# opencb/hpg-variant

Measured on AMD Instinct MI355X. Metric: variants/s chi2 assoc, higher is better.
Workload: dtype u8

## Files before the change

### hpg-variant_amd/csrc/hpgv_capi.hip

```cpp
#include "hpgv_internal.h"
#include <cstdlib>

extern "C" {

const char *hpgv_version(void) { return "hpgv-mi355x 0.1 (gfx950)"; }

int hpgv_device_count(void) {
    int n = 0;
    if (hipGetDeviceCount(&n) != hipSuccess) return -1;
    return n;
}

const char *hpgv_last_error(const hpgv_ctx *ctx) { return ctx ? ctx->err.c_str() : g_create_error.c_str(); }

static void read_environment(hpgv_ctx *ctx) {
    auto num = [](const char *name, long lo, long hi, long *out) { const char *e = getenv(name); if (e && *e) { long v = atol(e); *out = v < lo ? lo : v > hi ? hi : v; } };
    num("HPGV_BATCH_COPY", 0, 1, &ctx->batch_copy);
    num("HPGV_BATCH_FUSED", 0, 1, &ctx->batch_fused);
    num("HPGV_STATS_ALL2", 0, 1, &ctx->stats_all2);
    num("HPGV_ASSOC_ROWS", 0, 1, &ctx->assoc_rows);
    num("HPGV_PINNED_NONCOHERENT", 0, 1, &ctx->pinned_noncoherent);
    num("HPGV_VMM_TRACE", 0, 1, &ctx->vmm_trace);
    num("HPGV_DECODE_TILES", 0, 1, &ctx->decode_tiles);
#ifdef HPGV_ABLATION
// ... 120 lines not shown
    }
    ctx->tok_scratch.clear();
    for (auto &r : ctx->grow) grow_release(r);
    ctx->grow.clear();
    hpgv_epi_release(ctx->epi);
    for (Slot *s : ctx->slots) {
        s->release();
        if (s->stream) (void)hipStreamDestroy(s->stream);
        delete s;
    }
    for (int i = 0; i < 4; ++i) if (ctx->ev[i]) (void)hipEventDestroy(ctx->ev[i]);
    delete ctx;
}

#ifdef HPGV_ABLATION
#define HPGV_SHIPPED_ONLY(ok, what)
#else
#define HPGV_SHIPPED_ONLY(ok, what) if (!(ok)) return fail(ctx, HPGV_ERR_UNSUPPORTED, what ": that form is an ablation build's (-DHPGV_ABLATION, tools/build_ablation.py)");
#endif

int hpgv_set_option(hpgv_ctx *ctx, const char *key, long value) {
    if (is_group(ctx) && key && !strcmp(key, "group_self_exchange")) { ctx->group_self_exchange = value ? 1 : 0; return HPGV_OK; }
    GROUP_ALL(ctx, hpgv_set_option(m_, key, value))
    if (!ctx || !key) return HPGV_ERR_INVALID;
    if (!strcmp(key, "row_align")) {
        if (value < 16 || (value & (value - 1))) return fail(ctx, HPGV_ERR_INVALID, "row_align must be a power of two >= 16");
        if (ctx->assoc.set || ctx->tdt.set || ctx->stats.set)
            return fail(ctx, HPGV_ERR_STATE, "row_align must be set before the cohort");
        ctx->row_align = value;
    } else if (!strcmp(key, "row_pad")) {
        if (value < 0 || value % 16 || value > 65536) return fail(ctx, HPGV_ERR_INVALID, "row_pad must be a multiple of 16 in [0, 65536]");
        if (ctx->assoc.set || ctx->tdt.set || ctx->stats.set)
            return fail(ctx, HPGV_ERR_STATE, "row_pad must be set before the cohort");
        ctx->row_pad = value;
    } else if (!strcmp(key, "variants_per_wave")) {
        if (value < 1 || value > 1024) return fail(ctx, HPGV_ERR_INVALID, "variants_per_wave out of range");
        ctx->vpw = value;
    } else if (!strcmp(key, "nontemporal")) {
        HPGV_SHIPPED_ONLY(value != 0, "nontemporal = 0")
        ctx->nontemporal = value ? 1 : 0;
    } else if (!strcmp(key, "profile")) {
        ctx->profile = value ? 1 : 0;
    } else if (!strcmp(key, "scan_unroll")) {
        if (value != 4 && value != 8 && value != 10 && value != 12 && value != 16)
            return fail(ctx, HPGV_ERR_INVALID, "scan_unroll must be one of 4, 8, 10, 12, 16");
        HPGV_SHIPPED_ONLY(value == 4, "scan_unroll other than 4")
        ctx->scan_unroll = value;
    } else if (!strcmp(key, "pipeline")) {
        HPGV_SHIPPED_ONLY(value != 0, "pipeline = 0")
        ctx->pipeline = value ? 1 : 0;
    } else if (!strcmp(key, "fisher_cut_exp")) {
        if (value < 12 || value > 300) return fail(ctx, HPGV_ERR_INVALID, "fisher_cut_exp must be in [12, 300]");
        ctx->fisher_cut_exp = value;
    } else if (!strcmp(key, "epi_complete")) {
        ctx->epi_complete = value ? 1 : 0;
    } else if (!strcmp(key, "epi_triples_mfma")) {
        ctx->epi_triples_mfma = value ? 1 : 0;
    } else if (!strcmp(key, "epi_pairs_mfma")) {
        ctx->epi_pairs_mfma = value ? 1 : 0;
    } else if (!strcmp(key, "epi_wide")) {
        if (value < 0 || value > 2) return fail(ctx, HPGV_ERR_INVALID, "epi_wide must be 0 (the packed kernels' limits), 1 (the wide kernel where the shape needs it) or 2 (the wide kernel for every listed-combination launch)");
        ctx->epi_wide = value;
    } else if (!strcmp(key, "epi_triples_1pass")) {
        if (value < 0 || value > 2) return fail(ctx, HPGV_ERR_INVALID, "epi_triples_1pass must be 0 (two passes), 1 (the cells nine at a time) or 2 (one pass, one wave per SIMD)");
        HPGV_SHIPPED_ONLY(value != 2, "epi_triples_1pass = 2")
        ctx->epi_triples_1pass = value;
    } else if (!strcmp(key, "scan_lds")) {
        if (value < 0 || value > 160 * 1024) return fail(ctx, HPGV_ERR_INVALID, "scan_lds must be in [0, 163840]");
        ctx->scan_lds = value;
    } else if (!strcmp(key, "batch_copy")) {
        ctx->batch_copy = value ? 1 : 0;
    } else if (!strcmp(key, "inflate_wave")) {
        if (value < 0 || value > 4) return fail(ctx, HPGV_ERR_INVALID, "inflate_wave must be 0 (lane per block), 1 (by the number of blocks), 2 (wave per block), 4 (wave per block, several symbols per round) or 3 (lane per block, symbol tables in LDS)");
        HPGV_SHIPPED_ONLY(value == 1 || value == 4, "inflate_wave other than 1 / 4 (a wave per block, several symbols per round)")
        ctx->inflate_wave = value;
    } else if (!strcmp(key, "tokenizer_tiles")) {
        if (value < 0 || value > 2) return fail(ctx, HPGV_ERR_INVALID, "tokenizer_tiles must be 2 (one sweep), 1 (two sweeps) or 0 (line by line)");
        HPGV_SHIPPED_ONLY(value == 1, "tokenizer_tiles other than 1 (two sweeps)")
        ctx->tokenizer_tiles = value;
    } else if (!strcmp(key, "fisher_width")) {
        if (value != 64 && value != 32 && value != 16 && value != 8) return fail(ctx, HPGV_ERR_INVALID, "fisher_width must be 64, 32, 16 or 8");
        HPGV_SHIPPED_ONLY(value == 16, "fisher_width other than 16")
        ctx->fisher_width = value;
    } else if (!strcmp(key, "batch_fused")) {
        ctx->batch_fused = value ? 1 : 0;
    } else if (!strcmp(key, "pipe_waves")) {
        if (value != 4 && value != 6 && value != 8) return fail(ctx, HPGV_ERR_INVALID, "pipe_waves must be 4, 6 or 8");
        HPGV_SHIPPED_ONLY(value == 4, "pipe_waves other than 4")
        ctx->pipe_waves = value;
    } else if (!strcmp(key, "persistent")) {
        HPGV_SHIPPED_ONLY(value == 0, "persistent = 1")
        ctx->persistent = value ? 1 : 0;
    } else if (!strcmp(key, "part_aligned_loads")) {
        HPGV_SHIPPED_ONLY(value == 0, "part_aligned_loads = 1")
        ctx->part_aligned = value ? 1 : 0;
    } else if (!strcmp(key, "blocks_per_cu")) {
        if (value < 1 || value > 8) return fail(ctx, HPGV_ERR_INVALID, "blocks_per_cu must be in 1..8");
        ctx->blocks_per_cu = value;
    } else {
        return fail(ctx, HPGV_ERR_INVALID, "unknown option '%s'", key);
    }
    return HPGV_OK;
}


int hpgv_set_cohort(hpgv_ctx *ctx, const uint8_t *condition, int n_samples) {
    HPGV_ABI_TRY
    GROUP_ALL(ctx, hpgv_set_cohort(m_, condition, n_samples))
    if (!ctx) return HPGV_ERR_INVALID;
    if (!condition || n_samples < 0) return fail(ctx, HPGV_ERR_INVALID, "bad cohort arguments");
    DeviceGuard g(ctx->device);
    int nA = 0, nU = 0;
    for (int j = 0; j < n_samples; ++j) {
        if (condition[j] == HPGV_COND_AFFECTED) nA++;
        else if (condition[j] == HPGV_COND_UNAFFECTED) nU++;
    }
    size_t segA = round_up((size_t)nA, 16), segU = round_up((size_t)nU, 16);
    size_t pitch = round_up(segA + segU, (size_t)ctx->row_align) + (size_t)ctx->row_pad;
    if (pitch == 0) pitch = (size_t)ctx->row_align;
    if (!pitch_supported(pitch)) return fail(ctx, HPGV_ERR_UNSUPPORTED, "cohort of %d samples exceeds the row-length limit", n_samples);
    Layout &L = ctx->assoc;
    L.n_samples = n_samples;
    L.pitch = pitch;
    L.col_of_pos.assign(pitch, -1);
    size_t a = 0, u = segA;
    for (int j = 0; j < n_samples; ++j) {
        if (condition[j] == HPGV_COND_AFFECTED) L.col_of_pos[a++] = j;
        else if (condition[j] == HPGV_COND_UNAFFECTED) L.col_of_pos[u++] = j;
    }
    ctx->nA = nA; ctx->nU = nU; ctx->chunksA = (int)(segA / 16);
    {
        std::vector<uint8_t> cond(round_up((size_t)n_samples, 16) + 16, (uint8_t)HPGV_COND_OTHER);
        for (int j = 0; j < n_samples; ++j) cond[(size_t)j] = condition[j] == HPGV_COND_AFFECTED ? 1 : condition[j] == HPGV_COND_UNAFFECTED ? 0 : 2;
        HIPCHK(ctx, ctx->d_cond.reserve(cond.size()));
        HIPCHK(ctx, hipMemcpy(ctx->d_cond.p, cond.data(), cond.size(), hipMemcpyHostToDevice));
    }
    return upload_layout(ctx, L);
    HPGV_ABI_CATCH(ctx)
}

int hpgv_assoc_layout(const hpgv_ctx *ctx, int *n_affected, int *n_unaffected, size_t *pitch) {
    ctx = first_member(ctx);
    if (!ctx) return HPGV_ERR_INVALID;
    if (!ctx->assoc.set) return fail(ctx, HPGV_ERR_STATE, "hpgv_set_cohort has not been called");
    if (n_affected) *n_affected = ctx->nA;
    if (n_unaffected) *n_unaffected = ctx->nU;
    if (pitch) *pitch = ctx->assoc.pitch;
    return HPGV_OK;
}

int hpgv_set_logfact(hpgv_ctx *ctx, const double *table, size_t n) {
    GROUP_ALL(ctx, hpgv_set_logfact(m_, table, n))
    if (!ctx) return HPGV_ERR_INVALID;
    if (!table || n == 0) return fail(ctx, HPGV_ERR_INVALID, "empty log-factorial table");
    DeviceGuard g(ctx->device);
    ctx->n_lf = 0;
    if (ctx->cap_lf < n) {
        if (ctx->d_lf_base) { (void)hipFree(ctx->d_lf_base); ctx->d_lf_base = nullptr; ctx->d_lf = nullptr; ctx->cap_lf = 0; }
        HIPCHK(ctx, hipMalloc(&ctx->d_lf_base, (n + 4) * sizeof(double)));
        HIPCHK(ctx, hipMemset(ctx->d_lf_base, 0, (n + 4) * sizeof(double)));
        ctx->d_lf = ctx->d_lf_base + 2;
        ctx->cap_lf = n;
    }
    HIPCHK(ctx, hipMemcpy(ctx->d_lf, table, n * sizeof(double), hipMemcpyHostToDevice));
    ctx->n_lf = n;
    return HPGV_OK;
// ... 415 lines not shown
```

### hpg-variant_amd/csrc/hpgv_internal.h

```cpp
#pragma once
#include "../../include/hpgv.h"
#include "hpgv_kernels.h"
#include "hpgv_tdt_stats_kernels.h"
#include "hpgv_epi_kernels.h"

#include <hip/hip_runtime.h>
#include <cctype>

#include <algorithm>
#include <atomic>
#include <cmath>
#include <cstdarg>
#include <cstdio>
#include <cstring>
#include <mutex>
#include <new>
#include <string>
#include <vector>

namespace { thread_local std::string g_create_error; }

struct DevBuf {
    void *p = nullptr;
    size_t cap = 0;
// ... 71 lines not shown
    }
};

struct TextMeta {
    char *base;
    size_t max_lines;
    TextMeta(const DevBuf &meta, int max_lines_) : base(meta.as<char>()), max_lines((size_t)max_lines_) {}
    static size_t bytes(int max_lines) { return 16 + ((size_t)max_lines + 2) * sizeof(uint64_t) + (size_t)max_lines * 10 * sizeof(uint32_t) + 16; }
    int *n_lines() const { return (int *)base; }
    unsigned long long *line_off() const { return (unsigned long long *)(base + 16); }
    uint32_t *field_off() const { return (uint32_t *)(base + 16 + (max_lines + 2) * sizeof(uint64_t)); }
};

struct Staged {
    const uint8_t *d_raw = nullptr;
    size_t raw_pitch = 0;
    const uint8_t *d_laid = nullptr;
    int which = 0;
    const uint8_t *d_isx = nullptr;
    int n = 0;
    size_t out_stride = 0;
    bool text = false;
};

struct EpiState {
    bool have_data = false, have_folds = false;
    int V = 0, nA = 0, nU = 0, num_folds = 0, W = 0, V_alloc = 0, n_chunks = 0;
    bool wide_only = false;
    int fold_cap = 0;
    int rank_fold_cap = 0;
    uint8_t *d_data = nullptr;
    uint32_t *d_planes = nullptr;
    uint32_t rev_off = 0;
    hpgv_epi_rank_info rank_info{};
    uint32_t *d_marg = nullptr;
    bool complete = false;
    hpgv::EpiChunk *d_chunks = nullptr;
    uint32_t *d_chunk_cls = nullptr;
    hpgv::EpiFold *d_folds = nullptr;
    uint32_t *d_group_w0 = nullptr;
    std::vector<int32_t> group_size;
    DevBuf cand;
    unsigned *d_cand_count = nullptr;
    unsigned cand_cap = 0;
    double *d_thr = nullptr;
    DevBuf tile_base;
};

struct hpgv_ctx {
    std::vector<hpgv_ctx *> members;
    hpgv_ctx *parent = nullptr;
    struct GroupState *grp = nullptr;
    long group_self_exchange = 0;
    std::atomic<unsigned> deal_next{0};
    std::atomic<int> in_flight{0};
    int device = 0;
    mutable std::string err;
    std::mutex mu;
    long row_align = 16;
    long row_pad = 0;
    long vpw = 2;
    long nontemporal = 1;
    long profile = 0;
    std::mutex alias_mu;
    std::vector<std::pair<const char *, const char *>> text_alias;
    struct TextTiles { const char *d_text, *d_base; const void *d_tiles; uint64_t n_tiles; };
    std::vector<TextTiles> text_tiles;
    struct TextHeld { const char *host_text; Slot *slot; const char *d_text; const unsigned long long *d_line_off; int n_lines; };
    std::vector<TextHeld> text_held;
    long part_aligned = 0;
    long scan_unroll = 4;
    long persistent = 0;
    long blocks_per_cu = 8;
    long pipeline = 1;
    long pipe_waves = 4;
    long fisher_cut_exp = 22;
    long epi_complete = 1;
    long epi_pairs_mfma = 1;
    long epi_triples_mfma = 1;
    long epi_wide = 0;
    long epi_triples_1pass = 1;
    long scan_lds = 0;
    long fisher_width = 16;
    long inflate_wave = 1;
    long tokenizer_tiles = 1;
    long batch_copy = 0;
    long batch_fused = 1;
    long batch_lds_max = 65536;
    long stats_all2 = 1;
    long assoc_rows = 1;
    long pinned_noncoherent = 0;
    long vmm_trace = 0;
    long decode_tiles = 1;
#ifdef HPGV_ABLATION
    long stats_rows = 0, stats_bs = 0, stats_debug = 0;
    long fisher_lds = 0;
    long inflate_lds_pad = 0, inflate_wave_wgs = 0, inflate_lane_wgs = 0;
#endif
    int n_cus = 256;
    Layout assoc;
    int nA = 0, nU = 0, chunksA = 0;
    DevBuf d_cond;
    Layout tdt;
    hpgv::TdtPlan tdt_plan;
    Layout stats;
    Layout sgroups;
    std::vector<uint32_t> sg_off;
    std::vector<int> sg_size;
    DevBuf d_sg_chunks;
    DevBuf d_group_of_col;
    bool all_grouped = false;
    Layout mendel;
    int mendel_trios = 0, mendel_pchunks = 0;
    hpgv::MendelLuts mendel_luts{};
    uint8_t *d_mendel_male = nullptr;
    double *d_lf = nullptr;
    double *d_lf_base = nullptr;
    size_t n_lf = 0;
    size_t cap_lf = 0;
    DevBuf d_thr;
    hipEvent_t ev[4] = {nullptr, nullptr, nullptr, nullptr};
    bool have_scan_ev = false, have_stats_ev = false;
    std::vector<Slot *> slots;
    uint32_t *d_sink = nullptr;
    uint32_t *d_crc_tab = nullptr;
    struct TokScratch {
        hipStream_t stream = nullptr;
        DevBuf blocks, line_off, extra;
    };
    std::mutex tok_mu;
    std::vector<TokScratch *> tok_scratch;
    struct GrowRange { char *base = nullptr; size_t reserved = 0, committed = 0; std::vector<hipMemGenericAllocationHandle_t> pieces; std::vector<size_t> sizes; };
    std::vector<GrowRange> grow;
    double filt_min_maf = -1.0, filt_max_missing = -1.0;
    long filt_max_mendel = -1;
    double filt_min_dom = -1.0, filt_min_rec = -1.0;
    std::mutex epi_mu;
    EpiState epi;
};

namespace {

[[maybe_unused]] int fail(const hpgv_ctx *ctx, int code, const char *fmt, ...) {
    char buf[512];
    va_list ap;
    va_start(ap, fmt);
    vsnprintf(buf, sizeof buf, fmt, ap);
    va_end(ap);
    if (ctx) {
        ctx->err = buf;
        if (ctx->parent) {
            std::lock_guard<std::mutex> lk(ctx->parent->mu);
            ctx->parent->err = buf;
        }
    } else g_create_error = buf;
    return code;
}

#define HPGV_ABI_TRY try {
#define HPGV_ABI_CATCH(ctx)                                                                         \
    } catch (const std::bad_alloc &) { return fail(ctx, HPGV_ERR_NOMEM, "out of host memory"); }     \
      catch (...) { return fail(ctx, HPGV_ERR_INVALID, "unexpected C++ exception inside the engine"); }

inline bool is_group(const hpgv_ctx *c) { return c && !c->members.empty(); }
inline hpgv_ctx *first_member(hpgv_ctx *c) { return is_group(c) ? c->members[0] : c; }
inline const hpgv_ctx *first_member(const hpgv_ctx *c) { return is_group(c) ? c->members[0] : c; }
// ... 136 lines not shown
```

### hpg-variant_amd/csrc/hpgv_kernels.h

```cpp
#pragma once
#include <hip/hip_runtime.h>
#include <stdint.h>

namespace hpgv {

__device__ __forceinline__ uint32_t nib_nonzero(uint32_t x) {
    uint32_t y = x | (x << 1);
    y = y | (y << 2);
    return y & 0x88888888u;
}
__device__ __forceinline__ uint32_t nib_not_f(uint32_t x) { return nib_nonzero(~x); }

__device__ __forceinline__ int wave_sum(int v) {
    v += __builtin_amdgcn_update_dpp(0, v, 0xB1, 0xF, 0xF, true);
    v += __builtin_amdgcn_update_dpp(0, v, 0x4E, 0xF, 0xF, true);
    v += __builtin_amdgcn_update_dpp(0, v, 0x141, 0xF, 0xF, true);
    v += __builtin_amdgcn_update_dpp(0, v, 0x140, 0xF, 0xF, true);
    return __builtin_amdgcn_readlane(v, 0) + __builtin_amdgcn_readlane(v, 16) +
           __builtin_amdgcn_readlane(v, 32) + __builtin_amdgcn_readlane(v, 48);
}

template <bool NT>
__device__ __forceinline__ uint4 load16(const uint4 *p);
template <bool NT>
// ... 159 lines not shown
    const uint8_t *g0 = gt + (size_t)v_begin * pitch;
    AssocAcc acc = {0u, 0u, 0u};
    uint4 qa[U], qb[U];
    assoc_issue_tile<NT, U>(qa, g0, pitch, 0, ipr, chunks, lane);
    for (int t = 0; t < n_tiles; t += 2) {
        if (t + 1 < n_tiles) assoc_issue_tile<NT, U>(qb, g0, pitch, t + 1, ipr, chunks, lane);
        acc = assoc_consume_tile<U>(qa, acc, t, ipr, v_begin, lane, chunksA, TA, TU, is_x, counts);
        if (t + 1 < n_tiles) {
            if (t + 2 < n_tiles) assoc_issue_tile<NT, U>(qa, g0, pitch, t + 2, ipr, chunks, lane);
            acc = assoc_consume_tile<U>(qb, acc, t + 1, ipr, v_begin, lane, chunksA, TA, TU, is_x, counts);
        }
    }
}

__device__ __forceinline__ double chisq_p_value(double x) {
    if (x != x) return x;
    if (x <= 0.0) return 1.0;
    const double y = x / 2.0;
    double P;
    if (y > 0.5) P = 1.0 - erfc(sqrt(y));
    else         P = erf(sqrt(y));
    return 1.0 - P;
}

__device__ __forceinline__ double assoc_odds(int A1, int A2, int U1, int U2) {
    return (A2 == 0 || U1 == 0) ? __builtin_nan("") : ((double)A1 / A2) * ((double)U2 / U1);
}

__device__ __forceinline__ double assoc_chisq_value(int a, int c, int b, int d) {
    const double total = a + c + b + d;
    const double t_aff = a + c, t_un = b + d, t_1 = a + b, t_2 = c + d;
    const double e_a1 = (t_aff * t_1) / total;
    const double e_a2 = (t_aff * t_2) / total;
    const double e_u1 = (t_un * t_1) / total;
    const double e_u2 = (t_un * t_2) / total;
    return ((a - e_a1) * (a - e_a1)) / e_a1 + ((c - e_a2) * (c - e_a2)) / e_a2 +
           ((b - e_u1) * (b - e_u1)) / e_u1 + ((d - e_u2) * (d - e_u2)) / e_u2;
}

static __global__ __launch_bounds__(256) void k_assoc_chisq(const int4 *__restrict__ counts, int n,
                                                     double *__restrict__ odds,
                                                     double *__restrict__ chisq,
                                                     double *__restrict__ pval) {
    const int i = blockIdx.x * blockDim.x + threadIdx.x;
    if (i >= n) return;
    const int4 c4 = counts[i];
    const int a = c4.x, c = c4.y, b = c4.z, d = c4.w;
    const double x = assoc_chisq_value(a, c, b, d);
    odds[i] = assoc_odds(a, c, b, d);
    chisq[i] = x;
    pval[i] = chisq_p_value(x);
}

__device__ __forceinline__ double wave_sum_f64(double v) {
#pragma unroll
    for (int off = 32; off > 0; off >>= 1) v += __shfl_xor(v, off);
    return v;
}
__device__ __forceinline__ double wave_max_f64(double v) {
#pragma unroll
    for (int off = 32; off > 0; off >>= 1) { const double o = __shfl_xor(v, off); v = o > v ? o : v; }
    return v;
}

__device__ const double k_exp2_j64[64] = {
    0x1.0000000000000p+0, 0x1.02c9a3e778061p+0, 0x1.059b0d3158574p+0, 0x1.0874518759bc8p+0,
    0x1.0b5586cf9890fp+0, 0x1.0e3ec32d3d1a2p+0, 0x1.11301d0125b51p+0, 0x1.1429aaea92de0p+0,
    0x1.172b83c7d517bp+0, 0x1.1a35beb6fcb75p+0, 0x1.1d4873168b9aap+0, 0x1.2063b88628cd6p+0,
    0x1.2387a6e756238p+0, 0x1.26b4565e27cddp+0, 0x1.29e9df51fdee1p+0, 0x1.2d285a6e4030bp+0,
    0x1.306fe0a31b715p+0, 0x1.33c08b26416ffp+0, 0x1.371a7373aa9cbp+0, 0x1.3a7db34e59ff7p+0,
    0x1.3dea64c123422p+0, 0x1.4160a21f72e2ap+0, 0x1.44e086061892dp+0, 0x1.486a2b5c13cd0p+0,
    0x1.4bfdad5362a27p+0, 0x1.4f9b2769d2ca7p+0, 0x1.5342b569d4f82p+0, 0x1.56f4736b527dap+0,
    0x1.5ab07dd485429p+0, 0x1.5e76f15ad2148p+0, 0x1.6247eb03a5585p+0, 0x1.6623882552225p+0,
    0x1.6a09e667f3bcdp+0, 0x1.6dfb23c651a2fp+0, 0x1.71f75e8ec5f74p+0, 0x1.75feb564267c9p+0,
    0x1.7a11473eb0187p+0, 0x1.7e2f336cf4e62p+0, 0x1.82589994cce13p+0, 0x1.868d99b4492edp+0,
    0x1.8ace5422aa0dbp+0, 0x1.8f1ae99157736p+0, 0x1.93737b0cdc5e5p+0, 0x1.97d829fde4e50p+0,
    0x1.9c49182a3f090p+0, 0x1.a0c667b5de565p+0, 0x1.a5503b23e255dp+0, 0x1.a9e6b5579fdbfp+0,
    0x1.ae89f995ad3adp+0, 0x1.b33a2b84f15fbp+0, 0x1.b7f76f2fb5e47p+0, 0x1.bcc1e904bc1d2p+0,
    0x1.c199bdd85529cp+0, 0x1.c67f12e57d14bp+0, 0x1.cb720dcef9069p+0, 0x1.d072d4a07897cp+0,
    0x1.d5818dcfba487p+0, 0x1.da9e603db3285p+0, 0x1.dfc97337b9b5fp+0, 0x1.e502ee78b3ff6p+0,
    0x1.ea4afa2a490dap+0, 0x1.efa1bee615a27p+0, 0x1.f50765b6e4540p+0, 0x1.fa7c1819e90d8p+0,
};
__device__ __forceinline__ double fisher_exp(double e, const double *tab ) {
    const double kf = __builtin_rint(e * 0x1.71547652b82fep+6);
    double r = __builtin_fma(-kf, 0x1.62e42fe000000p-7, e);
    r = __builtin_fma(-kf, 0x1.f473de6af278fp-36, r);
    const int ki = (int)kf;
    const double tj = tab[ki & 63];
    double q = __builtin_fma(r, 1.0 / 120.0, 1.0 / 24.0);
    q = __builtin_fma(r, q, 1.0 / 6.0);
    q = __builtin_fma(r, q, 0.5);
    q = __builtin_fma(r * r, q, r);
    const double y = __builtin_fma(tj, q, tj);
    return e < -1100.0 ? 0.0 : __builtin_ldexp(y, ki >> 6);
}

struct FisherTab {
    const double *lf; const double *xt ; double konst; int r1, c1, d0;
    __device__ __forceinline__ double at(uint32_t byte_off) const { return *reinterpret_cast<const double *>(reinterpret_cast<const char *>(lf) + byte_off); }
    __device__ __forceinline__ double e(int x) const {
        const uint32_t x8 = (uint32_t)x << 3;
        return konst - at(x8) - at(((uint32_t)r1 << 3) - x8) - at(((uint32_t)c1 << 3) - x8) - at(((uint32_t)d0 << 3) + x8);
    }
    __device__ __forceinline__ double p(int x) const { return fisher_exp(e(x), xt); }
    __device__ __forceinline__ void e2(int x, double *e0, double *e1) const {
        const char *b = reinterpret_cast<const char *>(lf) - 16;
        double2 q0, q1, q2, q3;
        __builtin_memcpy(&q0, b + ((uint32_t)(x + 2) << 3), 16);
        __builtin_memcpy(&q1, b + ((uint32_t)(r1 - x + 1) << 3), 16);
        __builtin_memcpy(&q2, b + ((uint32_t)(c1 - x + 1) << 3), 16);
        __builtin_memcpy(&q3, b + ((uint32_t)(d0 + x + 2) << 3), 16);
        *e0 = konst - q0.x - q1.y - q2.y - q3.x;
        *e1 = konst - q0.y - q1.x - q2.x - q3.y;
    }
};

template <int W> __device__ __forceinline__ int sub_lane(int lane) { return lane & (W - 1); }
template <int W> __device__ __forceinline__ uint64_t sub_ballot(bool pred, int lane) {
    const uint64_t b = __ballot(pred);
    if constexpr (W == 64) { (void)lane; return b; }
    else return (b >> (lane & ~(W - 1))) & ((1ull << W) - 1ull);
}
template <int W> __device__ __forceinline__ double sub_sum_f64(double v) {
#pragma unroll
    for (int off = W / 2; off > 0; off >>= 1) v += __shfl_xor(v, off);
    return v;
}
template <int W> __device__ __forceinline__ double sub_first_f64(double v, int lane) { return __shfl(v, lane & ~(W - 1)); }

template <int W>
__device__ __forceinline__ void fisher_boundaries(const FisherTab &T, double thr , int L1, int R1, int L2, int R2, int lane,
                                                  int *xL, int *xR) {
    const int sl = sub_lane<W>(lane);
    while (R1 - L1 > W || R2 - L2 > W) {
        const bool go1 = R1 - L1 > W, go2 = R2 - L2 > W;
        const int step1 = (R1 - L1 + W - 1) / W, step2 = (R2 - L2 + W - 1) / W;
        const int x1 = L1 + sl * step1, x2 = L2 + sl * step2;
        const double v1 = (go1 && x1 < R1) ? T.e(x1) : 0.0;
        const double v2 = (go2 && x2 < R2) ? T.e(x2) : 0.0;
        if (go1) {
            const int j = __builtin_popcountll(sub_ballot<W>(x1 < R1 && v1 <= thr, lane));
            const int xj = L1 + j * step1;
            const int nL = (j == 0) ? L1 : L1 + (j - 1) * step1 + 1, nR = (j == W || xj >= R1) ? R1 : xj;
            L1 = nL; R1 = nR;
        }
        if (go2) {
            const int j = __builtin_popcountll(sub_ballot<W>(x2 < R2 && v2 > thr, lane));
            const int xj = L2 + j * step2;
            const int nL = (j == 0) ? L2 : L2 + (j - 1) * step2 + 1, nR = (j == W || xj >= R2) ? R2 : xj;
            L2 = nL; R2 = nR;
        }
    }
    const int x1 = L1 + sl, x2 = L2 + sl;
    const double v1 = x1 < R1 ? T.e(x1) : 0.0, v2 = x2 < R2 ? T.e(x2) : 0.0;
    *xL = L1 + __builtin_popcountll(sub_ballot<W>(x1 < R1 && v1 <= thr, lane));
    *xR = L2 + __builtin_popcountll(sub_ballot<W>(x2 < R2 && v2 > thr, lane));
}

template <int W>
__device__ __forceinline__ double fisher_tails(const FisherTab &T, int xL, int xR, int lo, int hi, int lane, double rel_cut) {
    const int sl = sub_lane<W>(lane);
    double partL = 0.0, partR = 0.0, cutL = 0.0, cutR = 0.0;
    bool onL = true, onR = true;
    for (int k = 0; onL || onR; ++k) {
        const int firstL = xL - 1 - 2 * W * k, firstR = xR + 2 * W * k;
        if (firstL < lo) onL = false;
        if (firstR > hi) onR = false;
        const int a = firstL - 2 * sl, b = firstR + 2 * sl;
        double eL0 = -2000.0, eL1 = -2000.0, eR0 = -2000.0, eR1 = -2000.0;
        if (onL && a >= lo) { double lo_e, hi_e; T.e2(a - 1, &lo_e, &hi_e); eL0 = hi_e; if (a - 1 >= lo) eL1 = lo_e; }
        if (onR && b <= hi) { double lo_e, hi_e; T.e2(b, &lo_e, &hi_e); eR0 = lo_e; if (b + 1 <= hi) eR1 = hi_e; }
        const double sL0 = fisher_exp(eL0, T.xt), sL1 = fisher_exp(eL1, T.xt), sR0 = fisher_exp(eR0, T.xt), sR1 = fisher_exp(eR1, T.xt);
        partL += sL0 + sL1; partR += sR0 + sR1;
        if (k == 0) { cutL = rel_cut * sub_first_f64<W>(sL0, lane); cutR = rel_cut * sub_first_f64<W>(sR0, lane); }
        if (onL && sub_ballot<W>(sL0 > cutL || sL1 > cutL, lane) == 0ull) onL = false;
        if (onR && sub_ballot<W>(sR0 > cutR || sR1 > cutR, lane) == 0ull) onR = false;
    }
    return sub_sum_f64<W>(partL + partR);
}

template <int W>
__device__ __forceinline__ bool fisher_boundary_windows(const FisherTab &T, double thr , int mode, int obs, int lane,
                                                        int *L1, int *R1, int *L2, int *R2) {
    const int sl = sub_lane<W>(lane);
    const int g1 = obs <= mode ? obs + 1 : 2 * mode - obs + 1, g2 = obs <= mode ? 2 * mode - obs : obs;
    int w1 = g1 - W / 2, w2 = g2 - W / 2;
    w1 = w1 > *R1 - W ? *R1 - W : w1; w1 = w1 < *L1 ? *L1 : w1;
    w2 = w2 > *R2 - W ? *R2 - W : w2; w2 = w2 < *L2 ? *L2 : w2;
    const int x1 = w1 + sl, x2 = w2 + sl;
    const bool in1 = x1 < *R1, in2 = x2 < *R2;
    const double v1 = in1 ? T.e(x1) : 0.0, v2 = in2 ? T.e(x2) : 0.0;
    const int n1 = __builtin_popcountll(sub_ballot<W>(in1, lane)), n2 = __builtin_popcountll(sub_ballot<W>(in2, lane));
    const int c1 = __builtin_popcountll(sub_ballot<W>(in1 && v1 <= thr, lane)), c2 = __builtin_popcountll(sub_ballot<W>(in2 && v2 > thr, lane));
    bool ok = true;
    if (c1 == 0 && w1 > *L1) { *R1 = w1; ok = false; }
    else if (c1 == n1 && w1 + n1 < *R1) { *L1 = w1 + n1; ok = false; }
    else { *L1 = w1 + c1; *R1 = w1 + c1; }
    if (c2 == 0 && w2 > *L2) { *R2 = w2; ok = false; }
    else if (c2 == n2 && w2 + n2 < *R2) { *L2 = w2 + n2; ok = false; }
    else { *L2 = w2 + c2; *R2 = w2 + c2; }
    return ok;
}

template <int W>
__device__ __forceinline__ double fisher_sub(int a, int b, int c, int d, const double *__restrict__ lf,
                                             const double *exp_tab , double rel_cut, int lane) {
    const int sl = sub_lane<W>(lane);
    const int r1 = a + b, r2 = c + d, c1 = a + c, nn = r1 + r2;
    const int lo = (c1 - r2) > 0 ? (c1 - r2) : 0;
    const int hi = r1 < c1 ? r1 : c1;
    FisherTab T;
    T.lf = lf; T.xt = exp_tab; T.r1 = r1; T.c1 = c1; T.d0 = r2 - c1;
    T.konst = lf[r1] + lf[r2] + lf[c1] + lf[nn - c1] - lf[nn];
    const double thr = T.e(a) + 9.9999995000000333e-08;
    double sum;
    if (hi - lo < 8 * W) {
        double part = 0.0;
        for (int x = lo + sl; x <= hi; x += W) {
            const double ex = T.e(x);
            if (ex <= thr) part += fisher_exp(ex, exp_tab);
        }
        sum = sub_sum_f64<W>(part);
    } else {
        const double prod = (double)(r1 + 1) * (double)(c1 + 1), den = (double)(nn + 2);
        double md = __builtin_floor(prod / den);
        const double rem = __builtin_fma(-md, den, prod);
        md += rem >= den ? 1.0 : (rem < 0.0 ? -1.0 : 0.0);
        int mode = (int)md;
        mode = mode < lo ? lo : (mode > hi ? hi : mode);
        int L1 = lo, R1 = mode + 1, L2 = mode + 1, R2 = hi + 1, xL, xR;
        if (fisher_boundary_windows<W>(T, thr, mode, a, lane, &L1, &R1, &L2, &R2)) { xL = L1; xR = L2; }
        else fisher_boundaries<W>(T, thr, L1, R1, L2, R2, lane, &xL, &xR);
        sum = fisher_tails<W>(T, xL, xR, lo, hi, lane, rel_cut);
    }
    return sum > 1.0 ? 1.0 : sum;
}

__device__ __forceinline__ double fisher_wave(int a, int b, int c, int d, const double *__restrict__ lf,
                                              const double *exp_tab , double rel_cut, int lane) {
    return fisher_sub<64>(a, b, c, d, lf, exp_tab, rel_cut, lane);
}

template <int W>
__global__ __launch_bounds__(256) void k_assoc_fisher(const int4 *__restrict__ counts, int n,
                                                      const double *__restrict__ lf,
                                                      double *__restrict__ odds,
                                                      double *__restrict__ pval, double rel_cut) {
    __shared__ double exp_tab[64];
    if (threadIdx.x < 64) exp_tab[threadIdx.x] = k_exp2_j64[threadIdx.x];
    __syncthreads();
    const int lane = threadIdx.x & 63;
    constexpr int PER_WAVE = 64 / W;
    const long wave = (long)blockIdx.x * (blockDim.x >> 6) + (threadIdx.x >> 6);
    const long v = wave * PER_WAVE + lane / W;
    if (v >= n) return;
    const int4 c4 = counts[v];
    const int a = c4.x, b = c4.y, c = c4.z, d = c4.w;
    const double p = fisher_sub<W>(a, b, c, d, lf, exp_tab, rel_cut, lane);
    if (sub_lane<W>(lane) == 0) {
        odds[v] = assoc_odds(a, b, c, d);
        pval[v] = p;
    }
}

__host__ __device__ __forceinline__ uint64_t splitmix64(uint64_t x) {
    x ^= x >> 30; x *= 0xbf58476d1ce4e5b9ULL;
    x ^= x >> 27; x *= 0x94d049bb133111ebULL;
    x ^= x >> 31;
    return x;
}
#define HPGV_SYNTH_SEED 0x4850475631ULL

static __global__ void k_synth_thresholds(uint64_t v0, int n, uint32_t *__restrict__ thr) {
    const int i = blockIdx.x * blockDim.x + threadIdx.x;
    if (i >= n) return;
    const uint64_t v = v0 + (uint64_t)i;
    const uint64_t h = splitmix64(HPGV_SYNTH_SEED ^ 0xA11E1EULL ^ v);
    const double u = (double)(h >> 11) * (1.0 / 9007199254740992.0);
    const double q = 0.05 + 0.45 * u;
    const uint32_t t_miss = 167772u;
    const double rest = (double)(16777216u - t_miss);
    const double omq = 1.0 - q;
    const double p00 = omq * omq;
    const double p01 = 2.0 * q * omq;
    const uint32_t t00 = t_miss + (uint32_t)floor(p00 * rest);
    const uint32_t t01 = t00 + (uint32_t)floor(p01 * rest);
    thr[3 * i + 0] = t_miss; thr[3 * i + 1] = t00; thr[3 * i + 2] = t01;
}

__device__ __forceinline__ uint32_t synth_gt(uint64_t vterm, uint64_t s, uint32_t tm, uint32_t t0,
                                             uint32_t t1) {
    const uint32_t r = (uint32_t)(splitmix64(vterm + s) >> 40);
    return (r < tm) ? 0xFFu : (r < t0) ? 0x00u : (r < t1) ? 0x01u : 0x11u;
}

enum { RECODE_NONE = 0, RECODE_TDT = 1, RECODE_STATS = 2, RECODE_MENDEL = 3, RECODE_EPI = 4 };

constexpr uint32_t TDT_F_UNUSABLE = 0x80u, TDT_M_UNUSABLE = 0x20u;
constexpr uint32_t TDT_C_INVALID = 4u;

__host__ __device__ __forceinline__ uint32_t tdt_parent_class(uint32_t g, uint32_t unusable) {
    const uint32_t a1 = g >> 4, a2 = g & 0xFu;
    if (a1 == 0xFu || a2 == 0xFu) return unusable;
    if (a1 && !a2) return unusable;
    if (!a1 && !a2) return 0u;
    if (!a1) return 1u;
    return (a1 == a2) ? 2u : 3u;
}
__host__ __device__ __forceinline__ uint32_t tdt_child_class(uint32_t g) {
    const uint32_t a1 = g >> 4, a2 = g & 0xFu;
    if (a1 == 0xFu || a2 == 0xFu) return TDT_C_INVALID;
    if (!a1 && !a2) return 0u;
    if (!a1) return 1u;
    if (!a2) return 2u;
    return 3u;
}
__host__ __device__ __forceinline__ uint32_t stats_flags(uint32_t g) {
    const uint32_t a1 = g >> 4, a2 = g & 0xFu;
    uint32_t f = 0;
    if (g == 0x00u) f |= 1u; else if (g == 0x01u) f |= 2u; else if (g == 0x10u) f |= 4u; else if (g == 0x11u) f |= 8u;
    if (a1 == 0xFu || a2 == 0xFu) f |= 0x10u;
    if (a1 == 0xFu && a2 == 0xFu) f |= 0x20u;
    if (!(f & 0xFu)) {
        if (a1 == 0u || a2 == 0u) f |= 0x40u;
        if (a1 == 1u || a2 == 1u) f |= 0x80u;
    }
    return f;
}

__host__ __device__ __forceinline__ uint32_t mendel_class(uint32_t g) {
    const uint32_t a1 = g >> 4, a2 = g & 0xFu;
    if (a1 == 0xFu || a2 == 0xFu) return 3u;
    if (!a1 && !a2) return 0u;
    return (a1 && a2) ? 2u : 1u;
}

__device__ __forceinline__ uint32_t recode_byte(uint32_t g, int mode, int p16, int pos, bool is_pad) {
    if (mode == RECODE_TDT) {
        if (p16 <= 0 || pos >= 3 * p16) return g;
        if (pos < p16) return tdt_parent_class(g, TDT_F_UNUSABLE);
        if (pos < 2 * p16) return tdt_parent_class(g, TDT_M_UNUSABLE);
        return tdt_child_class(g);
    }
    if (mode == RECODE_STATS) return is_pad ? 0u : stats_flags(g);
    if (mode == RECODE_MENDEL) return mendel_class(g);
    if (mode == RECODE_EPI) {
        const uint32_t a1 = g >> 4, a2 = g & 0xFu;
// ... 109 lines not shown
```

### hpg-variant_amd/csrc/hpgv_scan_capi.hip

```cpp
#include "hpgv_internal.h"
#include <type_traits>
#include "hpgv_inherit_kernels.h"

namespace {

unsigned scan_blocks(const hpgv_ctx *ctx, int n_variants) {
    const long waves = ((long)n_variants + ctx->vpw - 1) / ctx->vpw;
    return (unsigned)((waves + 3) / 4);
}

const char *const kAligned16 = "device buffers must be 16-byte aligned";
int scan_checks(hpgv_ctx *ctx, int n_variants, const void *d_gt, const void *d_out, uintptr_t out_mask, const char *align_text, bool *go) {
    *go = false;
    if (n_variants < 0 || (n_variants > 0 && (!d_gt || !d_out))) return fail(ctx, HPGV_ERR_INVALID, "bad scan arguments");
    if (n_variants == 0) return HPGV_OK;
    if (((uintptr_t)d_gt & 15) || ((uintptr_t)d_out & out_mask)) return fail(ctx, HPGV_ERR_INVALID, "%s", align_text);
    *go = true;
    return HPGV_OK;
}

template <typename F>
void launch_nt(const hpgv_ctx *ctx, F &&f) {
    if (ctx->nontemporal) f(std::true_type{}); else f(std::false_type{});
}
// ... 111 lines not shown


int hpgv_assoc_scan_dev(hpgv_ctx *ctx, const uint8_t *d_gt, int n_variants, const uint8_t *d_is_x,
                        int32_t *d_counts, void *stream) {
    ctx = first_member(ctx);
    if (!ctx) return HPGV_ERR_INVALID;
    if (!ctx->assoc.set) return fail(ctx, HPGV_ERR_STATE, "hpgv_set_cohort has not been called");
    bool go;
    if (const int rc = scan_checks(ctx, n_variants, d_gt, d_counts, 15, kAligned16, &go); rc || !go) return rc;
    DeviceGuard g(ctx->device);
    const Layout &L = ctx->assoc;
    const int vpw = (int)ctx->vpw;
    unsigned blocks = scan_blocks(ctx, n_variants);
    if (ctx->persistent) {
        const unsigned cap = (unsigned)(ctx->n_cus * ctx->blocks_per_cu);
        const unsigned need = (unsigned)(((long)n_variants + 3) / 4);
        blocks = need < cap ? need : cap;
    }
    hipStream_t st = (hipStream_t)stream;
    const uint8_t *gt = d_gt;
    int4 *out = (int4 *)d_counts;
    const int cA = ctx->chunksA, ch = L.chunks;
    const size_t pitch = L.pitch;
#define HPGV_LAUNCH_PIPE(NT, U, W)                                                                \
    hipLaunchKernelGGL((hpgv::k_assoc_scan_pipe<NT, U, W>), dim3(blocks), dim3(256), 0, st, gt, pitch, \
                       n_variants, cA, ch, d_is_x, out, vpw)
#ifndef HPGV_ABLATION
    return launch_profiled(ctx, st, 0, [&] { HPGV_LAUNCH_PIPE(true, 4, 4); });
#else
#define HPGV_LAUNCH_ASSOC(NT, U, S)                                                              \
    hipLaunchKernelGGL((hpgv::k_assoc_scan<NT, U, S>), dim3(blocks), dim3(256), 0, st, gt, pitch, \
                       n_variants, cA, ch, d_is_x, out, vpw)
#define HPGV_DISPATCH_U(NT, S)                                                                   \
    switch (ctx->scan_unroll) {                                                                  \
        case 4: HPGV_LAUNCH_ASSOC(NT, 4, S); break;                                              \
        case 10: HPGV_LAUNCH_ASSOC(NT, 10, S); break;                                            \
        case 12: HPGV_LAUNCH_ASSOC(NT, 12, S); break;                                            \
        case 16: HPGV_LAUNCH_ASSOC(NT, 16, S); break;                                            \
        default: HPGV_LAUNCH_ASSOC(NT, 8, S); break;                                             \
    }
#define HPGV_PIPE_W(NT, U)                                                                       \
    do {                                                                                         \
        if (ctx->pipe_waves == 8) { HPGV_LAUNCH_PIPE(NT, U, 8); }                                \
        else if (ctx->pipe_waves == 6) { HPGV_LAUNCH_PIPE(NT, U, 6); }                           \
        else { HPGV_LAUNCH_PIPE(NT, U, 4); }                                                     \
    } while (0)
    if (ctx->pipeline && !ctx->persistent)
        return launch_profiled(ctx, st, 0, [&] {
            if (ctx->nontemporal) {
                if (ctx->scan_unroll <= 4) HPGV_PIPE_W(true, 4); else HPGV_PIPE_W(true, 5);
            } else {
                if (ctx->scan_unroll <= 4) HPGV_PIPE_W(false, 4); else HPGV_PIPE_W(false, 5);
            }
        });
    return launch_profiled(ctx, st, 0, [&] {
        if (ctx->nontemporal) {
            if (ctx->persistent) { HPGV_DISPATCH_U(true, true) } else { HPGV_DISPATCH_U(true, false) }
        } else {
            if (ctx->persistent) { HPGV_DISPATCH_U(false, true) } else { HPGV_DISPATCH_U(false, false) }
        }
    });
#undef HPGV_DISPATCH_U
#undef HPGV_PIPE_W
#undef HPGV_LAUNCH_ASSOC
#endif
#undef HPGV_LAUNCH_PIPE
}

int hpgv_assoc_chisq_dev(hpgv_ctx *ctx, const int32_t *d_counts, int n_variants, double *d_odds,
                         double *d_chisq, double *d_p, void *stream) {
    ctx = first_member(ctx);
    if (!ctx) return HPGV_ERR_INVALID;
    if (n_variants < 0 || (n_variants > 0 && (!d_counts || !d_odds || !d_chisq || !d_p)))
        return fail(ctx, HPGV_ERR_INVALID, "bad chisq arguments");
    if (n_variants == 0) return HPGV_OK;
    DeviceGuard g(ctx->device);
    hipStream_t st = (hipStream_t)stream;
    return launch_profiled(ctx, st, 1, [&] {
        hipLaunchKernelGGL(hpgv::k_assoc_chisq, dim3((n_variants + 255) / 256), dim3(256), 0, st,
                           (const int4 *)d_counts, n_variants, d_odds, d_chisq, d_p);
    });
}

int hpgv_assoc_fisher_dev(hpgv_ctx *ctx, const int32_t *d_counts, int n_variants, double *d_odds,
                          double *d_p, void *stream) {
    ctx = first_member(ctx);
    if (!ctx) return HPGV_ERR_INVALID;
    if (n_variants < 0 || (n_variants > 0 && (!d_counts || !d_odds || !d_p)))
        return fail(ctx, HPGV_ERR_INVALID, "bad fisher arguments");
    if (const int rc = logfact_check(ctx)) return rc;
    if (n_variants == 0) return HPGV_OK;
    DeviceGuard g(ctx->device);
    hipStream_t st = (hipStream_t)stream;
    const double cut = pow(10.0, -(double)ctx->fisher_cut_exp);
    return launch_profiled(ctx, st, 1, [&] {
        const long per_block = 4 * (64 / ctx->fisher_width);
        const unsigned blocks = (unsigned)(((long)n_variants + per_block - 1) / per_block);
#ifdef HPGV_ABLATION
        const unsigned pad = (unsigned)ctx->fisher_lds;
        if (ctx->fisher_width == 64)
            hipLaunchKernelGGL(hpgv::k_assoc_fisher<64>, dim3(blocks), dim3(256), pad, st, (const int4 *)d_counts, n_variants, ctx->d_lf, d_odds, d_p, cut);
        else if (ctx->fisher_width == 8)
            hipLaunchKernelGGL(hpgv::k_assoc_fisher<8>, dim3(blocks), dim3(256), pad, st, (const int4 *)d_counts, n_variants, ctx->d_lf, d_odds, d_p, cut);
        else if (ctx->fisher_width == 32)
            hipLaunchKernelGGL(hpgv::k_assoc_fisher<32>, dim3(blocks), dim3(256), pad, st, (const int4 *)d_counts, n_variants, ctx->d_lf, d_odds, d_p, cut);
        else
#else
        const unsigned pad = 0u;
#endif
            hipLaunchKernelGGL(hpgv::k_assoc_fisher<16>, dim3(blocks), dim3(256), pad, st, (const int4 *)d_counts, n_variants, ctx->d_lf, d_odds, d_p, cut);
    });
}


int hpgv_tdt_scan_dev(hpgv_ctx *ctx, const uint8_t *d_gt, int n_variants, const uint8_t *d_is_x,
                      int32_t *d_tu, void *stream) {
    ctx = first_member(ctx);
    if (!ctx) return HPGV_ERR_INVALID;
    if (!ctx->tdt.set) return fail(ctx, HPGV_ERR_STATE, "hpgv_set_families has not been called");
    bool go;
    if (const int rc = scan_checks(ctx, n_variants, d_gt, d_tu, 7, "device buffers must be aligned", &go); rc || !go) return rc;
    DeviceGuard g(ctx->device);
    hipStream_t st = (hipStream_t)stream;
    return launch_profiled(ctx, st, 0, [&] {
        ctx->tdt_plan.launch_scan(d_gt, ctx->tdt.pitch, n_variants, d_is_x, (int2 *)d_tu,
                                  (int)ctx->vpw, ctx->nontemporal != 0, st);
    });
}

int hpgv_tdt_stats_dev(hpgv_ctx *ctx, const int32_t *d_tu, int n_variants, double *d_odds,
                       double *d_chisq, double *d_p, void *stream) {
    ctx = first_member(ctx);
    if (!ctx) return HPGV_ERR_INVALID;
    if (n_variants < 0 || (n_variants > 0 && (!d_tu || !d_odds || !d_chisq || !d_p)))
        return fail(ctx, HPGV_ERR_INVALID, "bad tdt stats arguments");
    if (n_variants == 0) return HPGV_OK;
    DeviceGuard g(ctx->device);
    hipStream_t st = (hipStream_t)stream;
    return launch_profiled(ctx, st, 1, [&] {
        hipLaunchKernelGGL(hpgv::k_tdt_stats, dim3((n_variants + 255) / 256), dim3(256), 0, st,
                           (const int2 *)d_tu, n_variants, d_odds, d_chisq, d_p);
    });
}


static int stats_scan(hpgv_ctx *ctx, const Layout &L, const uint8_t *d_gt, int n_variants, uint32_t off, int chunks, size_t lds,
                      int32_t *d_counts8, hipStream_t st) {
    bool go;
    if (const int rc = scan_checks(ctx, n_variants, d_gt, d_counts8, 15, kAligned16, &go); rc || !go) return rc;
    DeviceGuard g(ctx->device);
    const int vpw = (int)ctx->vpw;
    const unsigned blocks = scan_blocks(ctx, n_variants);
    return launch_profiled(ctx, st, 0, [&] {
        launch_nt(ctx, [&](auto NT) {
            constexpr bool nt = decltype(NT)::value;
            if (ctx->pipeline)
                hipLaunchKernelGGL((hpgv::k_stats_scan_hs<nt>), dim3(blocks), dim3(256), nt ? lds : 0, st, d_gt, L.pitch, n_variants, off, chunks, (int4 *)d_counts8, vpw);
            else
                hipLaunchKernelGGL((hpgv::k_stats_scan<nt, kScanUnroll>), dim3(blocks), dim3(256), 0, st, d_gt, L.pitch, n_variants, off, chunks, (int4 *)d_counts8, vpw);
        });
    });
}

int hpgv_stats_scan_dev(hpgv_ctx *ctx, const uint8_t *d_gt, int n_variants, int32_t *d_counts8, void *stream) {
    ctx = first_member(ctx);
    if (!ctx) return HPGV_ERR_INVALID;
    if (!ctx->stats.set) return fail(ctx, HPGV_ERR_STATE, "hpgv_set_stats_cohort has not been called");
    const Layout &L = ctx->stats;
    const size_t scan_lds = ctx->scan_lds > 0 ? (size_t)ctx->scan_lds : (L.pitch >= 6656 ? (size_t)49152 : (size_t)0);
    return stats_scan(ctx, L, d_gt, n_variants, 0u, L.chunks, scan_lds, d_counts8, (hipStream_t)stream);
}

int hpgv_stats_scan_group_dev(hpgv_ctx *ctx, const uint8_t *d_gt, int n_variants, int group, int32_t *d_counts8, void *stream) {
    ctx = first_member(ctx);
    if (!ctx) return HPGV_ERR_INVALID;
    if (!ctx->sgroups.set) return fail(ctx, HPGV_ERR_STATE, "hpgv_set_stats_groups has not been called");
    if (group < 0 || (size_t)group >= ctx->sg_off.size()) return fail(ctx, HPGV_ERR_INVALID, "group %d out of range", group);
// ... 168 lines not shown
```

Measured before the change: 136.5 million.

## Add blocked Fisher kernel with per-lane boundary search and dynamic subgroup tail scheduling

```diff
diff --git a/hpg-variant_amd/csrc/hpgv_capi.hip b/hpg-variant_amd/csrc/hpgv_capi.hip
--- a/hpg-variant_amd/csrc/hpgv_capi.hip
+++ b/hpg-variant_amd/csrc/hpgv_capi.hip
@@ -226,6 +226,10 @@
         if (value != 64 && value != 32 && value != 16 && value != 8) return fail(ctx, HPGV_ERR_INVALID, "fisher_width must be 64, 32, 16 or 8");
         HPGV_SHIPPED_ONLY(value == 16, "fisher_width other than 16")
         ctx->fisher_width = value;
+    } else if (!strcmp(key, "fisher_blocks")) {
+        if (value != 0 && value != 1 && value != 32 && value != 64) return fail(ctx, HPGV_ERR_INVALID, "fisher_blocks must be 0 (by the launch's size), 64 or 32 (variants per wave) or 1 (no blocks)");
+        HPGV_SHIPPED_ONLY(value == 0 || value == 32, "fisher_blocks other than 0 / 32")
+        ctx->fisher_blocks = value;
     } else if (!strcmp(key, "batch_fused")) {
         ctx->batch_fused = value ? 1 : 0;
     } else if (!strcmp(key, "pipe_waves")) {
diff --git a/hpg-variant_amd/csrc/hpgv_internal.h b/hpg-variant_amd/csrc/hpgv_internal.h
--- a/hpg-variant_amd/csrc/hpgv_internal.h
+++ b/hpg-variant_amd/csrc/hpgv_internal.h
@@ -177,6 +177,7 @@
     long epi_triples_1pass = 1;
     long scan_lds = 0;
     long fisher_width = 16;
+    long fisher_blocks = 0;
     long inflate_wave = 1;
     long tokenizer_tiles = 1;
     long batch_copy = 0;
diff --git a/hpg-variant_amd/csrc/hpgv_kernels.h b/hpg-variant_amd/csrc/hpgv_kernels.h
--- a/hpg-variant_amd/csrc/hpgv_kernels.h
+++ b/hpg-variant_amd/csrc/hpgv_kernels.h
@@ -265,6 +265,7 @@
     0x1.ea4afa2a490dap+0, 0x1.efa1bee615a27p+0, 0x1.f50765b6e4540p+0, 0x1.fa7c1819e90d8p+0,
 };
 __device__ __forceinline__ double fisher_exp(double e, const double *tab ) {
+    e = __builtin_fmax(e, -1100.0);
     const double kf = __builtin_rint(e * 0x1.71547652b82fep+6);
     double r = __builtin_fma(-kf, 0x1.62e42fe000000p-7, e);
     r = __builtin_fma(-kf, 0x1.f473de6af278fp-36, r);
@@ -275,7 +276,7 @@
     q = __builtin_fma(r, q, 0.5);
     q = __builtin_fma(r * r, q, r);
     const double y = __builtin_fma(tj, q, tj);
-    return e < -1100.0 ? 0.0 : __builtin_ldexp(y, ki >> 6);
+    return __builtin_ldexp(y, ki >> 6);
 }
 
 struct FisherTab {
@@ -340,26 +341,33 @@
     *xR = L2 + __builtin_popcountll(sub_ballot<W>(x2 < R2 && v2 > thr, lane));
 }
 
+struct FisherTails {
+    double partL, partR, cutL, cutR; int k; bool onL, onR;
+    __device__ __forceinline__ void start() { partL = partR = cutL = cutR = 0.0; k = 0; onL = onR = true; }
+};
+template <int W>
+__device__ __forceinline__ void fisher_turn(const FisherTab &T, int xL, int xR, int lo, int hi, int lane, double rel_cut, FisherTails &S) {
+    const int sl = sub_lane<W>(lane);
+    const int firstL = xL - 1 - 2 * W * S.k, firstR = xR + 2 * W * S.k;
+    if (firstL < lo) S.onL = false;
+    if (firstR > hi) S.onR = false;
+    const int a = firstL - 2 * sl, b = firstR + 2 * sl;
+    double eL0 = -2000.0, eL1 = -2000.0, eR0 = -2000.0, eR1 = -2000.0;
+    if (S.onL && a >= lo) { double lo_e, hi_e; T.e2(a - 1, &lo_e, &hi_e); eL0 = hi_e; if (a - 1 >= lo) eL1 = lo_e; }
+    if (S.onR && b <= hi) { double lo_e, hi_e; T.e2(b, &lo_e, &hi_e); eR0 = lo_e; if (b + 1 <= hi) eR1 = hi_e; }
+    const double sL0 = fisher_exp(eL0, T.xt), sL1 = fisher_exp(eL1, T.xt), sR0 = fisher_exp(eR0, T.xt), sR1 = fisher_exp(eR1, T.xt);
+    S.partL += sL0 + sL1; S.partR += sR0 + sR1;
+    if (S.k == 0) { S.cutL = rel_cut * sub_first_f64<W>(sL0, lane); S.cutR = rel_cut * sub_first_f64<W>(sR0, lane); }
+    if (S.onL && sub_ballot<W>(sL0 > S.cutL || sL1 > S.cutL, lane) == 0ull) S.onL = false;
+    if (S.onR && sub_ballot<W>(sR0 > S.cutR || sR1 > S.cutR, lane) == 0ull) S.onR = false;
+    ++S.k;
+}
 template <int W>
 __device__ __forceinline__ double fisher_tails(const FisherTab &T, int xL, int xR, int lo, int hi, int lane, double rel_cut) {
-    const int sl = sub_lane<W>(lane);
-    double partL = 0.0, partR = 0.0, cutL = 0.0, cutR = 0.0;
-    bool onL = true, onR = true;
-    for (int k = 0; onL || onR; ++k) {
-        const int firstL = xL - 1 - 2 * W * k, firstR = xR + 2 * W * k;
-        if (firstL < lo) onL = false;
-        if (firstR > hi) onR = false;
-        const int a = firstL - 2 * sl, b = firstR + 2 * sl;
-        double eL0 = -2000.0, eL1 = -2000.0, eR0 = -2000.0, eR1 = -2000.0;
-        if (onL && a >= lo) { double lo_e, hi_e; T.e2(a - 1, &lo_e, &hi_e); eL0 = hi_e; if (a - 1 >= lo) eL1 = lo_e; }
-        if (onR && b <= hi) { double lo_e, hi_e; T.e2(b, &lo_e, &hi_e); eR0 = lo_e; if (b + 1 <= hi) eR1 = hi_e; }
-        const double sL0 = fisher_exp(eL0, T.xt), sL1 = fisher_exp(eL1, T.xt), sR0 = fisher_exp(eR0, T.xt), sR1 = fisher_exp(eR1, T.xt);
-        partL += sL0 + sL1; partR += sR0 + sR1;
-        if (k == 0) { cutL = rel_cut * sub_first_f64<W>(sL0, lane); cutR = rel_cut * sub_first_f64<W>(sR0, lane); }
-        if (onL && sub_ballot<W>(sL0 > cutL || sL1 > cutL, lane) == 0ull) onL = false;
-        if (onR && sub_ballot<W>(sR0 > cutR || sR1 > cutR, lane) == 0ull) onR = false;
-    }
-    return sub_sum_f64<W>(partL + partR);
+    FisherTails S;
+    S.start();
+    while (S.onL || S.onR) fisher_turn<W>(T, xL, xR, lo, hi, lane, rel_cut, S);
+    return sub_sum_f64<W>(S.partL + S.partR);
 }
 
 template <int W>
@@ -385,6 +393,15 @@
     return ok;
 }
 
+__device__ __forceinline__ int fisher_mode(int r1, int c1, int nn, int lo, int hi) {
+    const double prod = (double)(r1 + 1) * (double)(c1 + 1), den = (double)(nn + 2);
+    double md = __builtin_floor(prod / den);
+    const double rem = __builtin_fma(-md, den, prod);
+    md += rem >= den ? 1.0 : (rem < 0.0 ? -1.0 : 0.0);
+    const int mode = (int)md;
+    return mode < lo ? lo : (mode > hi ? hi : mode);
+}
+
 template <int W>
 __device__ __forceinline__ double fisher_sub(int a, int b, int c, int d, const double *__restrict__ lf,
                                              const double *exp_tab , double rel_cut, int lane) {
@@ -405,12 +422,7 @@
         }
         sum = sub_sum_f64<W>(part);
     } else {
-        const double prod = (double)(r1 + 1) * (double)(c1 + 1), den = (double)(nn + 2);
-        double md = __builtin_floor(prod / den);
-        const double rem = __builtin_fma(-md, den, prod);
-        md += rem >= den ? 1.0 : (rem < 0.0 ? -1.0 : 0.0);
-        int mode = (int)md;
-        mode = mode < lo ? lo : (mode > hi ? hi : mode);
+        const int mode = fisher_mode(r1, c1, nn, lo, hi);
         int L1 = lo, R1 = mode + 1, L2 = mode + 1, R2 = hi + 1, xL, xR;
         if (fisher_boundary_windows<W>(T, thr, mode, a, lane, &L1, &R1, &L2, &R2)) { xL = L1; xR = L2; }
         else fisher_boundaries<W>(T, thr, L1, R1, L2, R2, lane, &xL, &xR);
@@ -446,6 +458,136 @@
     }
 }
 
+
+__device__ __forceinline__ void fisher_boundary_walk(const FisherTab &T, double thr , int mode, int obs, int lo, int hi,
+                                                     int *xL, int *xR) {
+    constexpr int WALK = 4;
+    int l1 = lo, h1 = mode + 1, l2 = mode + 1, h2 = hi + 1;
+    int p1 = obs <= mode ? obs + 1 : 2 * mode - obs + 1, p2 = obs <= mode ? 2 * mode - obs : obs;
+    for (int it = 0; l1 < h1 || l2 < h2; ++it) {
+        const bool go1 = l1 < h1, go2 = l2 < h2;
+        if (it >= WALK) { p1 = l1 + ((h1 - l1) >> 1); p2 = l2 + ((h2 - l2) >> 1); }
+        p1 = p1 > h1 - 1 ? h1 - 1 : p1; p1 = p1 < l1 ? l1 : p1;
+        p2 = p2 > h2 - 1 ? h2 - 1 : p2; p2 = p2 < l2 ? l2 : p2;
+        const double v1 = go1 ? T.e(p1) : 0.0, v2 = go2 ? T.e(p2) : 0.0;
+        if (go1) { if (v1 <= thr) { l1 = p1 + 1; p1 = l1; } else { h1 = p1; p1 = h1 - 1; } }
+        if (go2) { if (v2 > thr) { l2 = p2 + 1; p2 = l2; } else { h2 = p2; p2 = h2 - 1; } }
+    }
+    *xL = l1; *xR = l2;
+}
+
+template <int B> struct FisherBlock { double konst[B], p[B]; int r1[B], c1[B], d0[B], xL[B] , xR[B], lo[B], hi[B]; };
+
+__device__ __forceinline__ int fisher_pop(uint64_t &m) {
+    if (m == 0ull) return -1;
+    const int i = __builtin_ctzll(m);
+    m &= m - 1ull;
+    return i;
+}
+__device__ __forceinline__ void wave_lds_order() {
+    __builtin_amdgcn_fence(__ATOMIC_ACQ_REL, "wavefront");
+    __builtin_amdgcn_wave_barrier();
+}
+
+template <int B>
+__global__ __launch_bounds__(256) void k_assoc_fisher_blocks(const int4 *__restrict__ counts, int n,
+                                                             const double *__restrict__ lf,
+                                                             double *__restrict__ odds,
+                                                             double *__restrict__ pval, double rel_cut) {
+    static_assert(B == 64 || B == 32, "a lane per variant in phase A");
+    constexpr int W = 16;
+    __shared__ double exp_tab[64];
+    __shared__ FisherBlock<B> blocks[4];
+    if (threadIdx.x < 64) exp_tab[threadIdx.x] = k_exp2_j64[threadIdx.x];
+    __syncthreads();
+    const int lane = threadIdx.x & 63, sl = lane & (W - 1), sub = lane / W;
+    FisherBlock<B> &K = blocks[threadIdx.x >> 6];
+    const long v = ((long)blockIdx.x * (blockDim.x >> 6) + (threadIdx.x >> 6)) * B + lane;
+    const bool valid = lane < B && v < n;
+
+    bool whole;
+    {
+        int4 c4 = make_int4(0, 0, 0, 0);
+        if (valid) c4 = counts[v];
+        const int a = c4.x, b = c4.y, c = c4.z, d = c4.w;
+        const int r1 = a + b, r2 = c + d, c1 = a + c, nn = r1 + r2;
+        const int lo = (c1 - r2) > 0 ? (c1 - r2) : 0;
+        const int hi = r1 < c1 ? r1 : c1;
+        FisherTab T;
+        T.lf = lf; T.xt = exp_tab; T.r1 = r1; T.c1 = c1; T.d0 = r2 - c1;
+        T.konst = lf[r1] + lf[r2] + lf[c1] + lf[nn - c1] - lf[nn];
+        whole = hi - lo < 8 * W;
+        int xL = a, xR = 0;
+        if (!whole) {
+            const double thr = T.e(a) + 9.9999995000000333e-08;
+            fisher_boundary_walk(T, thr, fisher_mode(r1, c1, nn, lo, hi), a, lo, hi, &xL, &xR);
+        }
+        if (valid) {
+            K.konst[lane] = T.konst; K.r1[lane] = r1; K.c1[lane] = c1; K.d0[lane] = T.d0;
+            K.xL[lane] = xL; K.xR[lane] = xR; K.lo[lane] = lo; K.hi[lane] = hi;
+            odds[v] = assoc_odds(a, b, c, d);
+        }
+    }
+    wave_lds_order();
+    uint64_t todo = __ballot(valid && !whole), todo_whole = __ballot(valid && whole);
+
+    FisherTab T;
+    T.lf = lf; T.xt = exp_tab; T.r1 = T.c1 = T.d0 = 0; T.konst = 0.0;
+    FisherTails S;
+    S.start();
+    S.onL = S.onR = false;
+    int vi = -1, xL = 0, xR = 0, lo = 0, hi = 0;
+    bool want = true;
+    for (;;) {
+        const uint64_t fin = __ballot(want);
+        if (fin != 0ull) {
+            const double sum = sub_sum_f64<W>(S.partL + S.partR);
+            if (want && vi >= 0 && sl == 0) K.p[vi] = sum > 1.0 ? 1.0 : sum;
+            const int f0 = (int)(fin & 1ull), f1 = (int)((fin >> W) & 1ull), f2 = (int)((fin >> 2 * W) & 1ull), f3 = (int)((fin >> 3 * W) & 1ull);
+            uint64_t t = todo;
+            const int n0 = fisher_pop(t); const uint64_t t1 = t;
+            const int n1 = fisher_pop(t); const uint64_t t2 = t;
+            const int n2 = fisher_pop(t); const uint64_t t3 = t;
+            const int n3 = fisher_pop(t);
+            const int nfin = f0 + f1 + f2 + f3;
+            todo = nfin == 1 ? t1 : nfin == 2 ? t2 : nfin == 3 ? t3 : t;
+            const int rank = (sub > 0 ? f0 : 0) + (sub > 1 ? f1 : 0) + (sub > 2 ? f2 : 0);
+            if (want) {
+                vi = rank == 0 ? n0 : rank == 1 ? n1 : rank == 2 ? n2 : n3;
+                S.start();
+                if (vi >= 0) {
+                    T.konst = K.konst[vi]; T.r1 = K.r1[vi]; T.c1 = K.c1[vi]; T.d0 = K.d0[vi];
+                    xL = K.xL[vi]; xR = K.xR[vi]; lo = K.lo[vi]; hi = K.hi[vi];
+                } else {
+                    S.onL = S.onR = false;
+                }
+            }
+            if (__ballot(vi >= 0) == 0ull) break;
+        }
+        fisher_turn<W>(T, xL, xR, lo, hi, lane, rel_cut, S);
+        want = vi >= 0 && !(S.onL || S.onR);
+    }
+
+    while (todo_whole != 0ull) {
+        const int n0 = fisher_pop(todo_whole), n1 = fisher_pop(todo_whole), n2 = fisher_pop(todo_whole), n3 = fisher_pop(todo_whole);
+        const int wi = sub == 0 ? n0 : sub == 1 ? n1 : sub == 2 ? n2 : n3;
+        double part = 0.0;
+        if (wi >= 0) {
+            T.konst = K.konst[wi]; T.r1 = K.r1[wi]; T.c1 = K.c1[wi]; T.d0 = K.d0[wi];
+            const int whi = K.hi[wi];
+            const double thr = T.e(K.xL[wi]) + 9.9999995000000333e-08;
+            for (int x = K.lo[wi] + sl; x <= whi; x += W) {
+                const double ex = T.e(x);
+                if (ex <= thr) part += fisher_exp(ex, exp_tab);
+            }
+        }
+        const double sum = sub_sum_f64<W>(part);
+        if (wi >= 0 && sl == 0) K.p[wi] = sum > 1.0 ? 1.0 : sum;
+    }
+    wave_lds_order();
+    if (valid) pval[v] = K.p[lane];
+}
+
 __host__ __device__ __forceinline__ uint64_t splitmix64(uint64_t x) {
     x ^= x >> 30; x *= 0xbf58476d1ce4e5b9ULL;
     x ^= x >> 27; x *= 0x94d049bb133111ebULL;
diff --git a/hpg-variant_amd/csrc/hpgv_scan_capi.hip b/hpg-variant_amd/csrc/hpgv_scan_capi.hip
--- a/hpg-variant_amd/csrc/hpgv_scan_capi.hip
+++ b/hpg-variant_amd/csrc/hpgv_scan_capi.hip
@@ -217,6 +217,8 @@
     });
 }
 
+constexpr int kFisherBlocksMin = 12288 * 32;
+
 int hpgv_assoc_fisher_dev(hpgv_ctx *ctx, const int32_t *d_counts, int n_variants, double *d_odds,
                           double *d_p, void *stream) {
     ctx = first_member(ctx);
@@ -228,6 +230,17 @@
     DeviceGuard g(ctx->device);
     hipStream_t st = (hipStream_t)stream;
     const double cut = pow(10.0, -(double)ctx->fisher_cut_exp);
+    long blk = ctx->fisher_blocks;
+    if (blk == 0) blk = n_variants >= kFisherBlocksMin ? 32 : 1;
+    if (ctx->fisher_width != 16) blk = 1;
+    if (blk > 1)
+        return launch_profiled(ctx, st, 1, [&] {
+            const unsigned blocks = (unsigned)(((long)n_variants + 4 * blk - 1) / (4 * blk));
+            if (blk == 64)
+                hipLaunchKernelGGL(hpgv::k_assoc_fisher_blocks<64>, dim3(blocks), dim3(256), 0, st, (const int4 *)d_counts, n_variants, ctx->d_lf, d_odds, d_p, cut);
+            else
+                hipLaunchKernelGGL(hpgv::k_assoc_fisher_blocks<32>, dim3(blocks), dim3(256), 0, st, (const int4 *)d_counts, n_variants, ctx->d_lf, d_odds, d_p, cut);
+        });
     return launch_profiled(ctx, st, 1, [&] {
         const long per_block = 4 * (64 / ctx->fisher_width);
         const unsigned blocks = (unsigned)(((long)n_variants + per_block - 1) / per_block);
```

Result: no change. 135.1 million, median of 2 (-1.1%).
